# C-bowman/inference-tools

Measured on AMD Instinct MI355X. Metric: GpRegressor fit+predict wall-time and GFLOP/s at N=16384, d=8; % fp64 MFMA peak, higher is better.
Workload: dtype f64

## Files before the change

include/gpmi.h:

```cpp
#ifndef GPMI_H
#define GPMI_H

#include <stdint.h>

#ifdef __cplusplus
extern "C" {
#endif

#define GPMI_VERSION 100

#define GPMI_KERNEL_SE 0
#define GPMI_KERNEL_RQ 1
#define GPMI_KERNEL_SUM 2

#define GPMI_OK 0
#define GPMI_ERR_ARG (-1)
#define GPMI_ERR_HIP (-2)
#define GPMI_ERR_NOMEM (-3)
#define GPMI_ERR_NODEVICE (-4)
#define GPMI_ERR_INTERNAL (-5)

typedef struct gpmi_ctx gpmi_ctx;

int gpmi_version(void);
// ... 173 lines not shown
int gpmi_hdi_columns(gpmi_ctx* ctx, int64_t n, int64_t m, int64_t row_stride, int64_t col_stride,
                     const double* sample_host, int n_frac, const int64_t* L_host, int64_t ws_bytes,
                     double* hdi_host , int32_t* flag_host );

int gpmi_acf_columns(gpmi_ctx* ctx, int64_t n, int64_t m, int64_t row_stride, int64_t col_stride,
                     const double* sample_host, int64_t ws_bytes, double* f0_host , double* sum_host ,
                     int64_t* cut_host , int32_t* flag_host );
int gpmi_acf_lag_blocks(int64_t n, int64_t cap, int64_t* starts_host, int64_t* count);

int gpmi_timer_start(gpmi_ctx* ctx);
int gpmi_timer_stop(gpmi_ctx* ctx, float* ms);
int gpmi_flow_task_lists(int m, int nwg, int64_t cap, int32_t* out, int64_t* ntasks);

#define GPMI_PROF_KBUILD 0
#define GPMI_PROF_SYRK 1
#define GPMI_PROF_PANEL 2
#define GPMI_PROF_SOLVE 3
#define GPMI_PROF_SYRK_REST 4
#define GPMI_PROF_TRSM 5
#define GPMI_PROF_SYRK_SLICE 6
#define GPMI_PROF_FLOW 7
#define GPMI_PROF_NCLASS 8
int gpmi_profile_enable(gpmi_ctx* ctx, int on);
int gpmi_profile_read(gpmi_ctx* ctx, int klass, int64_t* launches, double* ms, double* flops,
                      double* bytes);
int gpmi_profile_reset(gpmi_ctx* ctx);
int gpmi_profile_clock(gpmi_ctx* ctx, double* ghz);

int gpmi_dev_alloc(gpmi_ctx* ctx, int64_t bytes, void** ptr_dev);
int gpmi_dev_free(gpmi_ctx* ctx, void* ptr_dev);
int gpmi_dev_upload(gpmi_ctx* ctx, void* dst_dev, const void* src_host, int64_t bytes);
int gpmi_dev_download(gpmi_ctx* ctx, void* dst_host, const void* src_dev, int64_t bytes);
int gpmi_dev_potrf(gpmi_ctx* ctx, double* A_dev, int64_t n, int64_t ld, int* info);
int gpmi_dev_gemm_nt(gpmi_ctx* ctx, double* C_dev, int64_t ldc, const double* A_dev, int64_t lda,
                     const double* B_dev, int64_t ldb, int64_t m, int64_t n, int64_t k, int lower);

#ifdef __cplusplus
}
#endif
#endif
```

inference-tools_amd/csrc/api.hip:

```cpp
#include "api_internal.h"
#include <malloc.h>


thread_local std::string g_create_err;


int lane_streams(gpmi_ctx* c, Lane& L) {
  const size_t index = c->lanes.size() - 1;
  L.owns_stream = index < 2;
  if (!L.owns_stream) L.stream = c->lanes[index % 2].stream;
  if (L.owns_stream) HIPCHK(c, hipStreamCreateWithFlags(&L.stream, hipStreamNonBlocking));
  hipDeviceProp_t prop;
  HIPCHK(c, hipGetDeviceProperties(&prop, c->device));
  c->ncu = prop.multiProcessorCount;
  HIPCHK(c, hipEventCreateWithFlags(&L.ev_la, hipEventDisableTiming));
  HIPCHK(c, hipEventCreateWithFlags(&L.ev_panel, hipEventDisableTiming));
  HIPCHK(c, hipEventCreateWithFlags(&L.ev_join, hipEventDisableTiming));
  HIPCHK(c, hipEventCreateWithFlags(&L.ev_main, hipEventDisableTiming));
  HIPCHK(c, hipEventCreateWithFlags(&L.ev_slice, hipEventDisableTiming));
  return GPMI_OK;
}


bool ensure_masked_pair(gpmi_ctx* c, Lane& L, int k) {
  (void)c;
  return L.sp[k] != nullptr && L.su[k] != nullptr;
}


int lane_masked_streams(gpmi_ctx* c, Lane& L) {
  const int ncu = c->ncu;
  if (ncu < 64 || ncu % 32 != 0) return GPMI_OK;
  for (int k = 0; k < GPMI_NPAIRS; ++k) {
    if (const char* e = std::getenv("GPMI_PANEL_CUS")) {
      const int v = std::atoi(e);
      if (v >= 8 && v <= ncu / 2 && v % 8 == 0) c->pair_cus[k] = v;
    }
    std::vector<uint32_t> panel((size_t)ncu / 32, 0u), upd((size_t)ncu / 32, 0xffffffffu);
    for (int i = 0; i < c->pair_cus[k]; ++i) {
      panel[(size_t)i / 32] |= 1u << (i % 32);
      upd[(size_t)i / 32] &= ~(1u << (i % 32));
    }
    hipError_t e1 = hipExtStreamCreateWithCUMask(&L.sp[k], (uint32_t)panel.size(), panel.data());
    hipError_t e2 = e1 == hipSuccess ? hipExtStreamCreateWithCUMask(&L.su[k], (uint32_t)upd.size(), upd.data()) : e1;
    if (e1 != hipSuccess || e2 != hipSuccess) {
      static bool told = false;
      if (!told) {
        told = true;
        std::fprintf(stderr, "[gpmi] a CU-masked stream pair could not be created (%s): this evaluation lane runs without "
                             "look-ahead and without the flag-ordered tail\n", hipGetErrorString(e1 != hipSuccess ? e1 : e2));
      }
      if (L.sp[k]) (void)hipStreamDestroy(L.sp[k]);
// ... 18 lines not shown
    }
    L.owns_pair = false;
  }
  const int64_t nt = c->np / GPMI_NB;
  HIPCHK(c, hipMalloc(&L.A, sizeof(double) * c->np * c->ld));
  HIPCHK(c, hipMalloc(&L.invD, sizeof(double) * nt * GPMI_NB * GPMI_NB));
  ZERO_SYNC(c, L.invD, sizeof(double) * nt * GPMI_NB * GPMI_NB);
  HIPCHK(c, hipMalloc(&L.vec, sizeof(double) * 4 * c->np));
  HIPCHK(c, hipMalloc(&L.red, sizeof(double) * 2 * RED_SLOTS));
  HIPCHK(c, hipMalloc(&L.info, sizeof(int) * RED_SLOTS));
  HIPCHK(c, hipHostMalloc(&L.h_red, sizeof(double) * 2 * RED_SLOTS));
  HIPCHK(c, hipHostMalloc(&L.h_info, sizeof(int) * RED_SLOTS));
  return GPMI_OK;
}

#define DBG_FREE(msg) do { if (std::getenv("GPMI_DEBUG_FREE")) std::fprintf(stderr, "[free] %s\n", msg); } while (0)
void lane_free(Lane& L) {
  DBG_FREE("lane: sync main stream");
  if (L.stream) (void)hipStreamSynchronize(L.stream);
  DBG_FREE("lane: sync masked streams");
  if (!L.owns_pair)
    for (int k = 0; k < GPMI_NPAIRS; ++k) L.sp[k] = L.su[k] = nullptr;
  for (int k = 0; k < GPMI_NPAIRS; ++k) {
    if (L.sp[k]) (void)hipStreamSynchronize(L.sp[k]);
    if (L.su[k]) (void)hipStreamSynchronize(L.su[k]);
  }
  potrf_flow_free(L);
  DBG_FREE("lane: destroy events");
  if (L.ev_la) (void)hipEventDestroy(L.ev_la);
  if (L.ev_panel) (void)hipEventDestroy(L.ev_panel);
  if (L.ev_join) (void)hipEventDestroy(L.ev_join);
  if (L.ev_main) (void)hipEventDestroy(L.ev_main);
  if (L.ev_slice) (void)hipEventDestroy(L.ev_slice);
  DBG_FREE("lane: destroy masked streams");
  if (L.sp[0] || L.su[0]) {
    static const int pause_ms = [] {
      const char* e = std::getenv("GPMI_DESTROY_PAUSE_MS");
      return e ? std::atoi(e) : 50;
    }();
    std::this_thread::sleep_for(std::chrono::milliseconds(pause_ms));
  }
  for (int k = 0; k < GPMI_NPAIRS; ++k) {
    if (L.sp[k]) (void)hipStreamDestroy(L.sp[k]);
    if (L.su[k]) (void)hipStreamDestroy(L.su[k]);
  }
  DBG_FREE("lane: free buffers");
  if (L.A) (void)hipFree(L.A);
  if (L.B2) (void)hipFree(L.B2);
  if (L.inv2) (void)hipFree(L.inv2);
  if (L.inv2_t) (void)hipFree(L.inv2_t);
  if (L.gws) (void)hipFree(L.gws);
  if (L.invD) (void)hipFree(L.invD);
  if (L.vec) (void)hipFree(L.vec);
  if (L.red) (void)hipFree(L.red);
  if (L.info) (void)hipFree(L.info);
  if (L.h_red) (void)hipHostFree(L.h_red);
  if (L.h_info) (void)hipHostFree(L.h_info);
  DBG_FREE("lane: destroy main stream");
  if (L.stream && L.owns_stream) (void)hipStreamDestroy(L.stream);
  DBG_FREE("lane: done");
  L = Lane();
}

int ensure_lanes(gpmi_ctx* c, size_t count) {
  while (c->lanes.size() < count) {
    c->lanes.emplace_back();
// ... 154 lines not shown
                     c->np, c->np, m > 0);
  }
  launch_add_diag_vec(s, dst, c->ld, c->noise, mx.extra, c->n);
}

int enqueue_factor_and_forward(gpmi_ctx* c, Lane& L, const CovParams& p, const double* mu_dev,
                               double mu_const, int slot, bool allow_lookahead,
                               const MixEval* mix, bool prebuild_inv2, double* backward_out, double* early_identity) {
  hipStream_t s = L.stream;
  L.inv2_valid = false;
  potrf_pair_quiesce(L);
  HIPCHK(c, hipMemsetAsync(L.info + slot, 0, sizeof(int), s));
  if (mix) {
    build_mix_square(c, s, *mix, L.A, false);
  } else {
    hipStream_t su = (!c->ycov && !((c->prof_mask >> GPMI_PROF_KBUILD) & 1))
                         ? potrf_first_update_stream(c, L, c->np, allow_lookahead)
                         : nullptr;
    static const bool no_split = std::getenv("GPMI_KBUILD_NO_SPLIT") != nullptr;
    if (su && !no_split) {
      HIPCHK(c, hipEventRecord(L.ev_join, s));
      HIPCHK(c, hipStreamWaitEvent(su, L.ev_join, 0));
      launch_kbuild_square_part(s, p, c->x, c->n, c->np, c->noise, L.A, c->ld, 1, GPMI_OB);
      launch_kbuild_square_part(su, p, c->x, c->n, c->np, c->noise, L.A, c->ld, 2, GPMI_OB);
    } else {
      ProfScope ps(c, s, GPMI_PROF_KBUILD, 0.0, 4.0 * c->np * c->np);
      launch_kbuild_square(s, p, c->x, c->n, c->np, c->noise, L.A, c->ld, true);
    }
  }
  if (c->ycov) launch_add_full(s, L.A, c->ld, c->ycov, c->n);
  static const bool early_fill = !std::getenv("GPMI_EARLY_FILL") || std::atoi(std::getenv("GPMI_EARLY_FILL")) != 0;
  L.early = Lane::EarlyWork();
  L.early.pending = true;
  L.early.y = c->y;
  L.early.mu = mu_dev;
  L.early.mu_const = mu_const;
  L.early.r = L.vec + 2 * c->np;
  L.early.n = c->n;
  L.early.np = c->np;
  L.early.fill[0] = L.vec;
  L.early.fill[1] = backward_out;
  L.early.ident = early_identity;
  L.early.ident_ld = c->ld;
  L.identity_ready = false;
  if (!early_fill) L.early.pending = false;
  potrf_lower(c, L, L.A, c->np, c->ld, L.invD, L.info + slot, allow_lookahead);
  if (!early_fill) L.early.pending = true;
  lane_run_early(L, s);
  if (prebuild_inv2 && L.su[0] && c->np >= 4 * GPMI_OB) {
    HIPCHK(c, hipEventRecord(L.ev_join, s));
    HIPCHK(c, hipStreamWaitEvent(L.su[0], L.ev_join, 0));
    if (int rc = ensure_inv2(c, L, L.su[0])) return rc;
    HIPCHK(c, hipEventRecord(L.ev_main, L.su[0]));
  }
  trsv_forward(c, s, L.A, c->np, c->ld, L.invD, L.vec + 2 * c->np, L.vec, L.info + slot, BatchShape(), true);
  if (prebuild_inv2 && L.inv2_valid && L.su[0]) {
    HIPCHK(c, hipEventRecord(L.ev_la, s));
    HIPCHK(c, hipStreamWaitEvent(L.su[0], L.ev_la, 0));
    launch_lml_reduce(L.su[0], L.vec, L.A, c->ld, c->np, L.red + 2 * slot);
    HIPCHK(c, hipEventRecord(L.ev_main, L.su[0]));
  } else {
    launch_lml_reduce(s, L.vec, L.A, c->ld, c->np, L.red + 2 * slot);
  }
  HIPCHK(c, hipGetLastError());
  return GPMI_OK;
}

int ensure_second_matrix(gpmi_ctx* c, Lane& L) {
  if (!L.B2) HIPCHK(c, hipMalloc(&L.B2, sizeof(double) * c->np * c->ld));
  return GPMI_OK;
}

int ensure_inv2(gpmi_ctx* c, Lane& F, hipStream_t s) {
  if (F.inv2_valid) return GPMI_OK;
  const int64_t nob = (c->np / GPMI_NB + 3) / 4;
  if (!F.inv2) HIPCHK(c, hipMalloc(&F.inv2, sizeof(double) * nob * GPMI_OB * GPMI_OB));
  if (!F.inv2_t) HIPCHK(c, hipMalloc(&F.inv2_t, sizeof(double) * nob * 256 * 256));
  build_inv2(s, F.A, c->np, c->ld, F.invD, F.inv2, F.inv2_t);
  HIPCHK(c, hipGetLastError());
  F.inv2_valid = true;
  return GPMI_OK;
}

int ensure_trsm_panel(gpmi_ctx* c, int64_t rows) {
  if (rows <= c->trsm_panel_rows) return GPMI_OK;
  if (c->trsm_panel) (void)hipFree(c->trsm_panel);
  c->trsm_panel = nullptr;
  c->trsm_panel_rows = 0;
// ... 549 lines not shown
    HIPCHK(c, hipMemcpyAsync(dbg + 22, &magic, sizeof(magic), hipMemcpyHostToDevice, s));
    launch_potrf_diag(s, A, ld, invD, dinfo, 0, dbg);
    std::vector<unsigned long long> hw(GPMI_STAMP_WORDS + TRACE_WORDS);
    HIPCHK(c, hipStreamSynchronize(s));
    HIPCHK(c, hipMemcpy(hw.data(), dbg, hw.size() * sizeof(unsigned long long), hipMemcpyDeviceToHost));
    const unsigned long long* h = hw.data() + 16;
    std::fprintf(stderr, "[potrf_diag] %.2f us | wave 0 cycles: load %llu | waits for its two tiles %llu | sub-diagonal panel + trailing tile %llu | end %llu | factor16 x8 %llu\n",
                 (double)(hw[8] - hw[0]) * 0.01, h[0], h[1], h[2], h[3], h[4]);
    for (int w = 0; w < 8; ++w) {
      if (w == 4) continue;
      std::fprintf(stderr, "[potrf_diag] wave %d (%s):", w, w == 0 ? "chain: start, W published, tiles seen, next block ready" : w < 4 ? "factor: start, W seen, panel done, panels seen, updates done" : "inverse: start, W seen, row done, operands seen, sums done");
      for (int k = 0; k < 9; ++k) {
        std::fprintf(stderr, " |");
        for (int e = 0; e < 6; ++e) {
          const unsigned long long v = hw[GPMI_STAMP_WORDS + (w * 9 + k) * 6 + e];
          if (v) std::fprintf(stderr, " %llu", v);
        }
      }
      std::fprintf(stderr, "\n");
    }
    (void)hipFree(dbg);
  } else
  potrf_lower(c, c->lanes[0], A, n, ld, invD, dinfo);
  int h = 0;
  hipError_t e = hipMemcpyAsync(&h, dinfo, sizeof(int), hipMemcpyDeviceToHost, s);
  if (e == hipSuccess) e = hipStreamSynchronize(s);
  (void)hipFree(invD);
  (void)hipFree(dinfo);
  HIPCHK(c, e);
  if (info) *info = h;
  return GPMI_OK;
}

int gpmi_dev_gemm_nt(gpmi_ctx* c, double* C, int64_t ldc, const double* A, int64_t lda,
                     const double* B, int64_t ldb, int64_t m, int64_t n, int64_t k, int lower) {
  if (!c) return GPMI_ERR_ARG;
  ARGCHK(c, m % GPMI_NB == 0 && n % GPMI_NB == 0 && k % 16 == 0 && m > 0 && n > 0 && k > 0,
         "m, n must be multiples of 128 and k of 16");
  if (int rc = set_device(c)) return rc;
  hipStream_t s;
  if (int rc = dev_stream(c, &s)) return rc;
  {
    const double tiles = lower ? (double)(n / GPMI_NB) * (n / GPMI_NB + 1) / 2.0 +
                                     (double)(m / GPMI_NB - n / GPMI_NB) * (n / GPMI_NB)
                               : (double)(m / GPMI_NB) * (n / GPMI_NB);
    unsigned long long* stamp =
        prof_stamp_slot(c, tiles * 2.0 * GPMI_NB * GPMI_NB * k, tiles * 16.0 * GPMI_NB * GPMI_NB);
    launch_gemm_nt(s, lower ? TILES_LOWER : TILES_RECT, OP_SUB, C, ldc, A, lda, B, ldb,
                   (int)(m / GPMI_NB), (int)(n / GPMI_NB), (int)k, stamp);
  }
  HIPCHK(c, hipGetLastError());
  HIPCHK(c, hipStreamSynchronize(s));
  return GPMI_OK;
}

}
```

inference-tools_amd/csrc/gpmi_internal.h:

```cpp
#pragma once
#include <hip/hip_runtime.h>
#include <cstdint>
#include <string>
#include <vector>

#include "gpmi.h"

constexpr int GPMI_NB = 128;
constexpr int GPMI_MAX_D = 64;
constexpr int GPMI_INFO_FLOW_TIMEOUT = -6;
constexpr int GPMI_NPAIRS = 1;

typedef double d2_t __attribute__((ext_vector_type(2)));
typedef double d4_t __attribute__((ext_vector_type(4)));

static inline int64_t round_up(int64_t v, int64_t m) { return (v + m - 1) / m * m; }

struct KParams {
  int kernel;
  int d;
  double a2;
  double kappa;
  double extra_diag;
  double inv_l2[GPMI_MAX_D];
};

constexpr int GPMI_MAX_SUM = 4;
struct CovParams : KParams {
  int nk = 0;
  KParams comp[GPMI_MAX_SUM] = {};
  CovParams() : KParams{} {}
  explicit CovParams(const KParams& k) : KParams(k) {}
};

struct ProfSlot {
  hipEvent_t e0, e1;
  int klass;
  double flops, bytes;
};

struct Lane {
  hipStream_t stream = nullptr;
  bool owns_stream = true;
  hipStream_t sp[GPMI_NPAIRS] = {nullptr};
  hipStream_t su[GPMI_NPAIRS] = {nullptr};
  bool owns_pair = true;
  struct EarlyWork {
    bool pending = false;
    const double* y = nullptr;
    const double* mu = nullptr;
    double mu_const = 0.0;
    double* r = nullptr;
    int64_t n = 0, np = 0;
    double* fill[2] = {nullptr, nullptr};
    double* ident = nullptr;
    int64_t ident_ld = 0;
  } early;
  bool identity_ready = false;
  bool pair_checked = false;
  hipEvent_t ev_la = nullptr, ev_panel = nullptr, ev_join = nullptr, ev_main = nullptr, ev_slice = nullptr;
  double* A = nullptr;
  double* invD = nullptr;
  double* B2 = nullptr;
  double* inv2 = nullptr;
  double* inv2_t = nullptr;
  bool inv2_valid = false;
  double* gws = nullptr;
  int64_t gws_doubles = 0;
  double* vec = nullptr;
  double* red = nullptr;
  int* info = nullptr;
  double* h_red = nullptr;
  int* h_info = nullptr;
  void* flow_tasks = nullptr;
  int* flow_off = nullptr;
  int* flow_flags = nullptr;
  int flow_m = 0, flow_nwg = 0, flow_nlists = 0;
  int64_t flow_ntasks = 0;
  double flow_flops_update = 0.0, flow_flops_trsm = 0.0;
};

struct LinvState {
  int64_t m = 0, mp = 0, ldm = 0;
  double* A = nullptr;
  double* At = nullptr;
  double* y = nullptr;
  double* sig2 = nullptr;
  double* zero = nullptr;
  double* K = nullptr;
  double* T = nullptr;
  double* J = nullptr;
  double* J2 = nullptr;
  double* Q = nullptr;
// ... 211 lines not shown
void launch_gemm_nt_range(hipStream_t s, GemmTiles tiles, GemmOp op, double* C, int64_t ldc, const double* A,
                          int64_t lda, const double* B, int64_t ldb, int ntr, int ntc, int k, int64_t first,
                          int64_t count, unsigned long long* stamp = nullptr);

void launch_gemm(hipStream_t s, GemmTiles tiles, GemmOp op, bool b_kmajor, int kskip, double* C,
                 int64_t ldc, const double* A, int64_t lda, const double* B, int64_t ldb, int ntr,
                 int ntc, int k, unsigned long long* stamp = nullptr, const GemmBatch& bt = GemmBatch());

hipStream_t potrf_first_update_stream(gpmi_ctx* c, Lane& lane, int64_t np, bool allow_lookahead);
void potrf_pair_quiesce(Lane& lane);
void launch_potrf_diag(hipStream_t s, double* Ablk, int64_t ld, double* invD, int* info, int col0,
                       unsigned long long* dbg = nullptr, const BatchShape& bs = BatchShape(), int* pub = nullptr,
                       int pub_val = 0);
void launch_potrf_diag_fault(hipStream_t s, double* Ablk, int64_t ld, const BatchShape& bs = BatchShape());
void potrf_lower_batched(gpmi_ctx* c, hipStream_t s, double* A, int64_t np, int64_t ld, double* invD,
                         int* info, const BatchShape& bs);
void launch_kbuild_square_batched(hipStream_t s, int kernel, const KParams* pdev, int batch, const double* x,
                                  int64_t n, int64_t np, const double* noise, double* A, int64_t ld,
                                  int64_t stride, int d, int64_t noise_stride = 0);
void potrf_lower(gpmi_ctx* c, Lane& lane, double* A, int64_t np, int64_t ld, double* invD,
                 int* info, bool allow_lookahead = true);

bool potrf_flow_enabled(gpmi_ctx* c, Lane& lane, int m);
bool potrf_flow_tail(gpmi_ctx* c, Lane& lane, double* A, int64_t ld, double* invD, int* info, int nt, int t0);
void potrf_flow_free(Lane& lane);

void trsv_forward(gpmi_ctx* c, hipStream_t s, const double* L, int64_t np, int64_t ld,
                  const double* invD, const double* r, double* out, int* err = nullptr,
                  const BatchShape& bs = BatchShape(), bool prefilled = false);
void trsv_backward(gpmi_ctx* c, hipStream_t s, const double* L, int64_t np, int64_t ld,
                   const double* invD, const double* r, double* out, int* err = nullptr,
                   const BatchShape& bs = BatchShape(), bool prefilled = false);
void lane_run_early(Lane& lane, hipStream_t s);
void trsm_identity_batched(hipStream_t s, const double* L, int64_t np, int64_t ld, const double* invD, double* Q,
                           const BatchShape& bs);
constexpr int GPMI_OB = 512;
void build_inv2(hipStream_t s, const double* L, int64_t np, int64_t ld, const double* invD, double* inv2,
                double* tmp);
void trsm_rows_forward(gpmi_ctx* c, hipStream_t s, const double* L, int64_t np, int64_t ld,
                       const double* inv2, double* Q, int64_t mp, bool upper_rhs, double* Qout,
                       double* panel);
void launch_set_identity(hipStream_t s, double* Q, int64_t ld, int64_t np, int batch = 1, int64_t sMat = 0);
void launch_copy(hipStream_t s, const double* src, double* dst, int64_t n);
void launch_copy_rows(hipStream_t s, const double* src, int64_t spitch, double* dst, int64_t dpitch, int64_t width,
                      int64_t height);
void launch_residual(hipStream_t s, const double* y, const double* mu, double mu_const, double* r,
                     int64_t n, int64_t np);
void launch_residual_batched(hipStream_t s, const double* y, const double* mus, const double* mu_consts,
                             double* r, int64_t n, int64_t np, const BatchShape& bs);
void launch_lml_reduce(hipStream_t s, const double* v, const double* L, int64_t ld, int64_t np,
                       double* red, const BatchShape& bs = BatchShape());
void launch_rows_dot(hipStream_t s, const double* Q, int64_t ld, int64_t mp, int64_t np,
                     const double* a, double* out, int batch = 1, int64_t sQ = 0, int64_t sVec = 0);
void launch_rows_sumsq(hipStream_t s, const double* Q, int64_t ld, int64_t mp, int64_t np,
                       double base, double* out, int batch = 1, int64_t sQ = 0, int64_t sVec = 0, double sign = 1.0);

void trsm_rows_backward(gpmi_ctx* c, hipStream_t s, const double* L, int64_t np, int64_t ld,
                        const double* invD, double* Q, int64_t mp, const double* inv2 = nullptr, double* panel = nullptr);

void launch_sd_reduce(hipStream_t s, const KParams& p, const double* x, int64_t n, const double* pts,
                      int64_t m, const double* Kq, int64_t ld, const double* W, int64_t ldw,
                      double scale, double* out);
void launch_grad_rhs(hipStream_t s, const KParams& p, const double* x, int64_t n, int64_t np,
                     const double* pts, int64_t rows_valid, int64_t rows_padded, const double* Kq,
                     int64_t ld, double* G);
void launch_grad_cov(hipStream_t s, const KParams& p, const double* G, int64_t ld, int64_t np,
// ... 2 lines not shown
```

inference-tools_amd/csrc/potrf.hip:

```cpp
#include <cstdlib>
#include <type_traits>
#include <utility>
#include <vector>

#include "gpmi_internal.h"
#include "potrf_diag.h"

namespace {

constexpr int NB = GPMI_NB;
using potrf_diag::DIAG_THREADS;

__global__ __launch_bounds__(DIAG_THREADS) void potrf_diag_kernel(double* __restrict__ A, int64_t ld,
                                                         double* __restrict__ invD,
                                                         int* __restrict__ info, int col0,
                                                         unsigned long long* __restrict__ dbg,
                                                         int64_t strideA, int64_t strideInv, int* pub, int pub_val) {
  if (pub && threadIdx.x == 0 && blockIdx.z == 0)
    __hip_atomic_store(pub, pub_val, __ATOMIC_RELAXED, __HIP_MEMORY_SCOPE_AGENT);
  __shared__ potrf_diag::DiagShared sh;
  potrf_diag::potrf_diag_body<false>(A + (int64_t)blockIdx.z * strideA, ld, invD + (int64_t)blockIdx.z * strideInv,
                                     info + blockIdx.z, col0, dbg, sh, potrf_diag::DiagPub());
}

}

namespace {
__global__ void fault_scale_kernel(double* A, int64_t ld, double f, int64_t strideA) {
  A += (int64_t)blockIdx.z * strideA;
  const int r = blockIdx.x, c = threadIdx.x;
  if (c <= r) A[(int64_t)r * ld + c] *= f;
}
}

void launch_potrf_diag_fault(hipStream_t s, double* Ablk, int64_t ld, const BatchShape& bs) {
  static const double fault = [] {
    const char* e = std::getenv("GPMI_FAULT_DIAG_EPS");
    return e ? std::atof(e) : 0.0;
  }();
  if (fault != 0.0)
    hipLaunchKernelGGL(fault_scale_kernel, dim3(NB, 1, (unsigned)bs.count), dim3(NB), 0, s, Ablk, ld, 1.0 + fault,
                       bs.sMat);
}

void launch_potrf_diag(hipStream_t s, double* Ablk, int64_t ld, double* invD, int* info, int col0,
                       unsigned long long* dbg, const BatchShape& bs, int* pub, int pub_val) {
  hipLaunchKernelGGL(potrf_diag_kernel, dim3(1, 1, (unsigned)bs.count), dim3(DIAG_THREADS), 0, s, Ablk, ld, invD,
                     info, col0, dbg, bs.sMat, bs.sInv, pub, pub_val);
  launch_potrf_diag_fault(s, Ablk, ld, bs);
}

namespace {

void factor_panel(gpmi_ctx* c, hipStream_t sp, double* A, int64_t ld, double* invD, int* info, int nt,
                  int J, int Je, int ncu = 0) {
  GemmBatch on;
  on.ncu_hint = ncu;
  on.b_lower_tri = true;
  static const bool trace = std::getenv("GPMI_CHAIN_TRACE") != nullptr;
  auto slot = [&](int tag) { return trace ? prof_stamp_slot(c, 0.0, 0.0, GPMI_PROF_NCLASS + tag) : nullptr; };
  for (int j = J; j < Je; ++j) {
    double* Ajj = A + (int64_t)j * NB * ld + (int64_t)j * NB;
    double* invDj = invD + (int64_t)j * NB * NB;
    const int below = nt - j - 1;
    {
      ProfScope ps(c, sp, GPMI_PROF_PANEL, (double)NB * NB * NB / 3.0 + 2.0 * below * NB * NB * NB,
                   8.0 * NB * NB * (2.0 + 2.0 * below));
      launch_potrf_diag(sp, Ajj, ld, invDj, info, j * NB, slot(0));
      if (below > 0) {
        double* A21 = Ajj + (int64_t)NB * ld;
        launch_gemm_nt(sp, TILES_RECT, OP_ASSIGN, A21, ld, A21, ld, invDj, NB, below, 1, NB, slot(1), on);
      }
    }
    const int pc = Je - j - 1;
    if (below > 0 && pc > 0) {
      double* A21 = Ajj + (int64_t)NB * ld;
      double* C = A21 + NB;
      const double tiles = pc * (pc + 1) / 2.0 + (double)(below - pc) * pc;
      ProfScope ps(c, sp, GPMI_PROF_PANEL, tiles * 2.0 * NB * NB * NB, tiles * 16.0 * NB * NB);
      launch_gemm_nt(sp, TILES_LOWER, OP_SUB, C, ld, A21, ld, A21, ld, below, pc, NB, slot(2));
    }
  }
}

void update_columns(gpmi_ctx* c, hipStream_t s, double* A, int64_t ld, int nt, int t0, int t1, int ka, int ke,
                    int ncu, int64_t slice = 0) {
  const int rows = nt - t0, cols = t1 - t0;
  const int kw = (ke - ka) * NB;
  if (rows <= 0 || cols <= 0 || kw <= 0) return;
  double* P = A + (int64_t)t0 * NB * ld + (int64_t)ka * NB;
  double* C = A + (int64_t)t0 * NB * ld + (int64_t)t0 * NB;
  const int64_t tiles = (int64_t)cols * (cols + 1) / 2 + (int64_t)(rows - cols) * cols - slice;
  const int64_t nfull = gemm_split_point(tiles, ncu, kw);
  static const int64_t BIG_MIN = [] {
    const char* e = std::getenv("GPMI_BIG_MIN");
    return (int64_t)(e ? std::atoi(e) : 384);
  }();
  const bool big = tiles >= BIG_MIN && kw > 128;
  int64_t nmain = big ? nfull : 0;
  if (big && nfull > 0 && nfull < tiles && gemm_mixed_launches()) nmain = tiles;
  unsigned long long* stamp = nullptr;
  unsigned long long* stamp_rest = nullptr;
  if (nmain > 0)
    stamp = prof_stamp_slot(c, (double)nmain * 2.0 * NB * NB * kw, (double)nmain * 16.0 * NB * NB + 8.0 * rows * NB * kw);
  if (tiles > nmain)
    stamp_rest = prof_stamp_slot(c, (double)(tiles - nmain) * 2.0 * NB * NB * kw, (double)(tiles - nmain) * 16.0 * NB * NB,
                                 GPMI_PROF_SYRK_REST);
  if (big)
    launch_gemm_nt_split(s, TILES_LOWER, OP_SUB, C, ld, P, ld, P, ld, rows, cols, kw, nfull, stamp, stamp_rest, tiles);
  else
    launch_gemm_nt_split(s, TILES_LOWER, OP_SUB, C, ld, P, ld, P, ld, rows, cols, kw, nfull, stamp_rest, nullptr, tiles);
// ... 22 lines not shown
  const double per_main = tile_us / (2.0 * ncu_main), per_panel = tile_us / (2.0 * ncu_panel);
  static const double CHAIN0 = [] {
    const char* e = std::getenv("GPMI_SLICE_CHAIN_US");
    return e ? std::atof(e) : 146.0;
  }();
  static const double SLOPE = [] {
    const char* e = std::getenv("GPMI_SLICE_CHAIN_SLOPE");
    return e ? std::atof(e) : 6.1;
  }();
  const double chain = CHAIN0 + SLOPE * rem;
  const double su = 20.0 + (double)(tiles_la + tiles_main) * per_main;
  double x = (su - chain) / (per_main + per_panel) * PCT / 100.0;
  const int64_t round = 2 * ncu_panel;
  int64_t n = x > 0 ? (int64_t)(x / round) * round : 0;
  const int64_t safe = tiles_main - (int64_t)8 * rem;
  if (n > safe) n = safe > 0 ? safe / round * round : 0;
  return n;
}

}

bool ensure_masked_pair(gpmi_ctx* c, Lane& L, int k);

namespace {
constexpr int OUTER_TILES = 4;
int lookahead_min() {
  static const int v = [] {
    const char* e = std::getenv("GPMI_LOOKAHEAD_MIN");
    const int x = e ? std::atoi(e) : 52;
    return x > 0 ? x : (1 << 30);
  }();
  return v;
}
}

void potrf_pair_quiesce(Lane& lane) {
  for (int k = 0; k < GPMI_NPAIRS; ++k)
    for (hipStream_t q : {lane.sp[k], lane.su[k]})
      if (q && hipStreamQuery(q) != hipSuccess) {
        (void)hipGetLastError();
        (void)hipStreamSynchronize(q);
      }
  lane.pair_checked = true;
}

hipStream_t potrf_first_update_stream(gpmi_ctx* c, Lane& lane, int64_t np, bool allow_lookahead) {
  const int nt = (int)(np / NB);
  if (!allow_lookahead || nt - OUTER_TILES < lookahead_min() || !ensure_masked_pair(c, lane, 0)) return nullptr;
  return lane.su[0];
}

void potrf_lower(gpmi_ctx* c, Lane& lane, double* A, int64_t np, int64_t ld, double* invD, int* info,
                 bool allow_lookahead) {
  hipStream_t sf = lane.stream;
  const int nt = (int)(np / NB);
  const int OBT = OUTER_TILES;
  const int LOOKAHEAD_MIN = lookahead_min();
  if (!lane.pair_checked) potrf_pair_quiesce(lane);
  lane.pair_checked = false;
  const bool la_ok = allow_lookahead && nt - OBT >= LOOKAHEAD_MIN && ensure_masked_pair(c, lane, 0);
  const bool flow_ok = allow_lookahead;
  if (flow_ok && !(la_ok && nt - OBT >= LOOKAHEAD_MIN) && potrf_flow_enabled(c, lane, nt) &&
      potrf_flow_tail(c, lane, A, ld, invD, info, nt, 0))
    return;
  auto follow = [](hipStream_t waiter, hipStream_t producer, hipEvent_t ev) {
    if (waiter != producer) (void)hipStreamWaitEvent(waiter, ev, 0);
  };
  auto tile0 = [&](int panel) { return panel * OBT < nt ? panel * OBT : nt; };
  const int NP = (nt + OBT - 1) / OBT;
  factor_panel(c, sf, A, ld, invD, info, nt, 0, tile0(1));
  hipStream_t panel_stream = sf;
  hipStream_t main_stream = sf;
  bool sliced = false;
  (void)hipEventRecord(lane.ev_panel, sf);
  (void)hipEventRecord(lane.ev_main, sf);
  if (la_ok && NP > 1 && nt - tile0(1) >= LOOKAHEAD_MIN) lane_run_early(lane, sf);
  for (int p = 0; p + 1 < NP; ++p) {
    const int k0 = tile0(p), k1 = tile0(p + 1);
    const int rem = nt - k1;
    const bool overlap = la_ok && rem >= LOOKAHEAD_MIN;
    hipStream_t su = overlap ? lane.su[0] : sf, sp = overlap ? lane.sp[0] : sf;
    const int ncu = overlap ? c->ncu - c->pair_cus[0] : c->ncu;
    follow(su, panel_stream, lane.ev_panel);
    follow(su, main_stream, lane.ev_main);
    int64_t slice = 0;
    if (overlap) {
      const int k2 = tile0(p + 2);
      update_columns(c, su, A, ld, nt, k1, k2, k0, k1, ncu);
      (void)hipEventRecord(lane.ev_la, su);
      (void)hipStreamWaitEvent(sp, lane.ev_la, 0);
      const int w = k2 - k1, r2 = nt - k2;
      slice = slice_tiles(rem, (int64_t)w * (w + 1) / 2 + (int64_t)(rem - w) * w, (int64_t)r2 * (r2 + 1) / 2,
                          (k1 - k0) * NB, ncu, c->pair_cus[0]);
      if (sliced) (void)hipStreamWaitEvent(su, lane.ev_slice, 0);
      update_columns(c, su, A, ld, nt, k2, nt, k0, k1, ncu, slice);
      (void)hipEventRecord(lane.ev_main, su);
    } else {
      if (sliced) (void)hipStreamWaitEvent(su, lane.ev_slice, 0);
      update_columns(c, su, A, ld, nt, k1, nt, k0, k1, ncu);
      if (flow_ok && potrf_flow_enabled(c, lane, nt - k1) && potrf_flow_tail(c, lane, A, ld, invD, info, nt, k1)) return;
    }
    sliced = false;
    main_stream = su;
    factor_panel(c, sp, A, ld, invD, info, nt, k1, tile0(p + 2), overlap ? c->pair_cus[0] : 0);
    if (overlap) (void)hipEventRecord(lane.ev_panel, sp);
    panel_stream = sp;
    if (slice > 0) {
      update_slice(c, sp, A, ld, nt, tile0(p + 2), nt, k0, k1, slice);
      (void)hipEventRecord(lane.ev_slice, sp);
      sliced = true;
    }
  }
  follow(sf, panel_stream, lane.ev_panel);
  follow(sf, main_stream, lane.ev_main);
  if (sliced) (void)hipStreamWaitEvent(sf, lane.ev_slice, 0);
}

void potrf_lower_batched(gpmi_ctx* c, hipStream_t s, double* A, int64_t np, int64_t ld, double* invD,
                         int* info, const BatchShape& bs) {
  (void)c;
  static const int OBT = [] {
    const char* e = std::getenv("GPMI_BATCH_OUTER");
    const int v = e ? std::atoi(e) : 4;
    return v > 0 ? v : 1;
  }();
  const int nt = (int)(np / NB);
  GemmBatch inplace{bs.count, bs.sMat, bs.sMat, bs.sInv};
  inplace.b_lower_tri = true;
  const GemmBatch upd{bs.count, bs.sMat, bs.sMat, bs.sMat};
  static const bool left = [] {
    const char* e = std::getenv("GPMI_BATCH_LEFT");
    return !e || std::atoi(e) != 0;
  }();
  for (int J = 0; J < nt; J += OBT) {
    const int Je = (J + OBT < nt) ? J + OBT : nt;
    for (int j = J; j < Je; ++j) {
      double* Ajj = A + (int64_t)j * NB * ld + (int64_t)j * NB;
      double* invDj = invD + (int64_t)j * NB * NB;
      const int below = nt - j - 1;
      if (left && j > J) {
        const double* P = A + (int64_t)j * NB * ld + (int64_t)J * NB;
        launch_gemm_nt(s, TILES_LOWER, OP_SUB, Ajj, ld, P, ld, P, ld, nt - j, 1, (j - J) * NB, nullptr, upd);
      }
      launch_potrf_diag(s, Ajj, ld, invDj, info, j * NB, nullptr, bs);
// ... 17 lines not shown
```

inference-tools_amd/csrc/solve.hip:

```cpp
#include <cstdlib>
#include <mutex>

#include "gpmi_internal.h"

namespace {

constexpr int NB = GPMI_NB;

__device__ inline double wave_sum(double v) {
#pragma unroll
  for (int off = 32; off > 0; off >>= 1) v += __shfl_down(v, off, 64);
  return v;
}

constexpr unsigned long long FLOW_SENTINEL = 0xFFF8DEADBEEF0000ull;
constexpr int FLOW_THREADS = 512;
constexpr int FLOW_SPIN_LIMIT = 1 << 22;

__device__ inline double flow_poll(const double* p, int* err, bool& dead) {
  const unsigned long long* q = reinterpret_cast<const unsigned long long*>(p);
  unsigned long long bits = __hip_atomic_load(q, __ATOMIC_RELAXED, __HIP_MEMORY_SCOPE_AGENT);
  int spins = 0;
  while (bits == FLOW_SENTINEL && !dead) {
    __builtin_amdgcn_s_sleep(1);
// ... 370 lines not shown
  }
  s = wave_sum(s);
  if (lane == 0) out[row] = sign * (base - s);
}

}

constexpr int64_t FLOW_GATE_MIN = 32;
namespace {
std::mutex g_sweep_mu;
hipEvent_t g_sweep_ev[64] = {nullptr};
bool g_sweep_used[64] = {false};
}
static void flow_gate_enter(gpmi_ctx* c, hipStream_t s, int64_t workgroups) {
  if (workgroups <= FLOW_GATE_MIN || c->device < 0 || c->device >= 64) return;
  std::lock_guard<std::mutex> lk(g_sweep_mu);
  const int d = c->device;
  if (!g_sweep_ev[d] && hipEventCreateWithFlags(&g_sweep_ev[d], hipEventDisableTiming) != hipSuccess) {
    g_sweep_ev[d] = nullptr;
    (void)hipGetLastError();
    return;
  }
  if (g_sweep_used[d]) (void)hipStreamWaitEvent(s, g_sweep_ev[d], 0);
}
static void flow_gate_leave(gpmi_ctx* c, hipStream_t s, int64_t workgroups) {
  if (workgroups <= FLOW_GATE_MIN || c->device < 0 || c->device >= 64) return;
  std::lock_guard<std::mutex> lk(g_sweep_mu);
  const int d = c->device;
  if (!g_sweep_ev[d]) return;
  (void)hipEventRecord(g_sweep_ev[d], s);
  g_sweep_used[d] = true;
}

void lane_run_early(Lane& lane, hipStream_t s) {
  Lane::EarlyWork& e = lane.early;
  if (!e.pending) return;
  e.pending = false;
  launch_residual(s, e.y, e.mu, e.mu_const, e.r, e.n, e.np);
  for (double* f : e.fill)
    if (f) hipLaunchKernelGGL(flow_fill_kernel, dim3((unsigned)((e.np + 255) / 256), 1, 1), dim3(256), 0, s, f, e.np, (int64_t)0);
  if (e.ident) {
    launch_set_identity(s, e.ident, e.ident_ld, e.np);
    lane.identity_ready = true;
  }
}

void trsv_forward(gpmi_ctx* c, hipStream_t s, const double* L, int64_t np, int64_t ld,
                  const double* invD, const double* r, double* out, int* err, const BatchShape& bs, bool prefilled) {
  const int nt = (int)(np / NB);
  flow_gate_enter(c, s, (int64_t)nt);
  ProfScope ps(c, s, GPMI_PROF_SOLVE, (double)np * np, 4.0 * np * np);
  if (!prefilled)
    hipLaunchKernelGGL(flow_fill_kernel, dim3((unsigned)((np + 255) / 256), 1, (unsigned)bs.count), dim3(256), 0, s,
                       out, np, bs.sVec);
  const unsigned grid = bs.count > 1 ? 8u * (unsigned)nt * (unsigned)((bs.count + 7) / 8) : (unsigned)nt;
  hipLaunchKernelGGL(trsv_fwd_flow_kernel, dim3(grid), dim3(FLOW_THREADS), 0, s, L, ld, invD, r, out, err, bs.sMat,
                     bs.sInv, bs.sVec, nt, bs.count);
  flow_gate_leave(c, s, (int64_t)nt);
}

void trsv_backward(gpmi_ctx* c, hipStream_t s, const double* L, int64_t np, int64_t ld,
                   const double* invD, const double* r, double* out, int* err, const BatchShape& bs, bool prefilled) {
  const int nt = (int)(np / NB);
  flow_gate_enter(c, s, (int64_t)nt);
  ProfScope ps(c, s, GPMI_PROF_SOLVE, (double)np * np, 4.0 * np * np);
  if (!prefilled)
    hipLaunchKernelGGL(flow_fill_kernel, dim3((unsigned)((np + 255) / 256), 1, (unsigned)bs.count), dim3(256), 0, s, out,
                       np, bs.sVec);
  const unsigned grid = bs.count > 1 ? 8u * (unsigned)nt * (unsigned)((bs.count + 7) / 8) : (unsigned)nt;
  hipLaunchKernelGGL(trsv_bwd_flow_kernel, dim3(grid), dim3(FLOW_THREADS), 0, s, L, ld, invD, r, out, err, nt, bs.sMat,
                     bs.sInv, bs.sVec, bs.count);
  flow_gate_leave(c, s, (int64_t)nt);
}

void build_inv2(hipStream_t s, const double* L, int64_t np, int64_t ld, const double* invD, double* inv2,
                double* tmp) {
  const int nt = (int)(np / NB);
// ... 168 lines not shown
```

inference-tools_amd/inference_amd/_lib.py:

```python
import atexit
import ctypes as C
import os
import sys
import weakref

import numpy as np

_HERE = os.path.dirname(os.path.abspath(__file__))
LIB_PATH = os.environ.get("GPMI_LIB") or os.path.join(_HERE, "lib", "libgpmi.so")

KERNEL_SE = 0
KERNEL_RQ = 1
KERNEL_SUM = 2
PROF_KBUILD, PROF_SYRK, PROF_PANEL, PROF_SOLVE, PROF_SYRK_REST, PROF_TRSM, PROF_SYRK_SLICE, PROF_FLOW = 0, 1, 2, 3, 4, 5, 6, 7
OPT_LOCKSTEP_ALWAYS, OPT_RESERVE_POINTS, OPT_NO_FLOW = 1, 2, 3
PREDICT_PANEL = 256
_TRACE_MS = float(os.environ["GPMI_TRACE_CALLS"]) if os.environ.get("GPMI_TRACE_CALLS") else None
ERR_INTERNAL = -5


class GpmiUnavailable(RuntimeError):
    """libgpmi.so (the HIP extension) or an MI355X device is missing."""


# ... 72 lines not shown
    "gpmi_comm_allgather": (C.c_int, [_vp, _dp, _dp, _i64]),
    "gpmi_comm_broadcast": (C.c_int, [_vp, _dp, _i64, C.c_int]),
    "gpmi_comm_count": (C.c_int, [_vp, C.POINTER(C.c_int)]),
    "gpmi_comm_destroy": (C.c_int, [_vp]),
    "gpmi_kde_create": (C.c_int, [_vp, _i64, _dp, _i64, C.POINTER(_i64), C.POINTER(_i64), C.POINTER(_vp)]),
    "gpmi_kde_destroy": (C.c_int, [_vp]),
    "gpmi_kde_eval": (C.c_int, [_vp, _i64, _dp, C.POINTER(_i64), C.c_double, _dp, _dp]),
    "gpmi_kde_cv_logprob": (C.c_int, [_vp, _i64, _dp, C.c_int, _dp, C.c_double, _dp]),
    "gpmi_kde2d_create": (C.c_int, [_vp, _i64, _dp, _dp, C.POINTER(_vp)]),
    "gpmi_kde2d_destroy": (C.c_int, [_vp, _vp]),
    "gpmi_kde2d_eval": (C.c_int, [_vp, _vp, _i64, _dp, _dp, C.c_double, C.c_double, _dp]),
    "gpmi_kde2d_self": (C.c_int, [_vp, _vp, C.c_double, C.c_double, _dp, C.POINTER(_i64)]),
    "gpmi_kde2d_grid": (C.c_int, [_vp, _vp, _i64, _dp, _i64, _dp, C.c_double, C.c_double, _dp]),
    "gpmi_unimodal_create": (C.c_int, [_vp, _i64, _dp, C.POINTER(_vp)]),
    "gpmi_unimodal_destroy": (C.c_int, [_vp, _vp]),
    "gpmi_unimodal_logpdf_sums": (C.c_int, [_vp, _vp, _i64, C.c_int, _dp, _dp]),
    "gpmi_hdi_columns": (C.c_int, [_vp, _i64, _i64, _i64, _i64, _dp, C.c_int, C.POINTER(_i64), _i64, _dp,
                                   C.POINTER(C.c_int32)]),
    "gpmi_acf_columns": (C.c_int, [_vp, _i64, _i64, _i64, _i64, _dp, _i64, _dp, _dp, C.POINTER(_i64),
                                   C.POINTER(C.c_int32)]),
    "gpmi_acf_lag_blocks": (C.c_int, [_i64, _i64, C.POINTER(_i64), C.POINTER(_i64)]),
    "gpmi_timer_start": (C.c_int, [_vp]),
    "gpmi_timer_stop": (C.c_int, [_vp, C.POINTER(C.c_float)]),
    "gpmi_profile_enable": (C.c_int, [_vp, C.c_int]),
    "gpmi_profile_read": (C.c_int, [_vp, C.c_int, C.POINTER(_i64), _dp, _dp, _dp]),
    "gpmi_profile_reset": (C.c_int, [_vp]),
    "gpmi_profile_clock": (C.c_int, [_vp, _dp]),
    "gpmi_dev_alloc": (C.c_int, [_vp, _i64, C.POINTER(_vp)]),
    "gpmi_dev_free": (C.c_int, [_vp, _vp]),
    "gpmi_dev_upload": (C.c_int, [_vp, _vp, _vp, _i64]),
    "gpmi_dev_download": (C.c_int, [_vp, _vp, _vp, _i64]),
    "gpmi_dev_potrf": (C.c_int, [_vp, _vp, _i64, _i64, _ip]),
    "gpmi_dev_gemm_nt": (C.c_int, [_vp, _vp, _i64, _vp, _i64, _vp, _i64, _i64, _i64, _i64, C.c_int]),
}

_lib = None


def load():
    global _lib
    if _lib is None:
        if not os.path.exists(LIB_PATH):
            raise GpmiUnavailable(
                f"{LIB_PATH} not found - build the HIP extension first "
                "(python -c 'import __graft_entry__ as g; g.build()' or make -C inference-tools_amd/csrc)"
            )
        lib = C.CDLL(LIB_PATH)
        for name, (res, args) in SIGNATURES.items():
            fn = getattr(lib, name)
            fn.restype = res
            fn.argtypes = args
        _lib = lib
        atexit.register(_close_all_handles)
    return _lib


def device_count() -> int:
    cnt = C.c_int(0)
    load().gpmi_device_count(C.byref(cnt))
    return cnt.value


def device_identity(device: int) -> str:
    buf = C.create_string_buffer(64)
    rc = load().gpmi_device_pci_bus_id(int(device), buf, 64)
    return buf.value.decode() if rc == 0 else ""
# ... 89 lines not shown
```

Before: 54920.

## Overlap forward triangular solve with Cholesky panels and split lookahead update

Adds a panel-forward kernel that solves the right-hand side against each finished Cholesky panel and updates the residual for the rows below. It runs on the factorization streams while later panels are still being factored, so the trailing forward trsv only covers the unfinished tiles. It also splits the lookahead column update so the next panel can start after its first tile column is ready, waiting on the rest later. This adds extra kernels, events and cross-stream dependencies, which brings synchronization overhead and a risk of ordering errors.

```diff
diff --git a/include/gpmi.h b/include/gpmi.h
--- a/include/gpmi.h
+++ b/include/gpmi.h
@@ -229,6 +229,9 @@
 int gpmi_dev_upload(gpmi_ctx* ctx, void* dst_dev, const void* src_host, int64_t bytes);
 int gpmi_dev_download(gpmi_ctx* ctx, void* dst_host, const void* src_dev, int64_t bytes);
 int gpmi_dev_potrf(gpmi_ctx* ctx, double* A_dev, int64_t n, int64_t ld, int* info);
+int gpmi_dev_panel_forward(gpmi_ctx* ctx, const double* L_dev, int64_t ld, const double* invD_dev, double* r_dev,
+                           double* z_dev, int64_t nt, int64_t k0, int64_t w, int64_t row_first, int64_t row_count,
+                           int store_z);
 int gpmi_dev_gemm_nt(gpmi_ctx* ctx, double* C_dev, int64_t ldc, const double* A_dev, int64_t lda,
                      const double* B_dev, int64_t ldb, int64_t m, int64_t n, int64_t k, int lower);
 
diff --git a/inference-tools_amd/csrc/api.hip b/inference-tools_amd/csrc/api.hip
--- a/inference-tools_amd/csrc/api.hip
+++ b/inference-tools_amd/csrc/api.hip
@@ -18,6 +18,8 @@
   HIPCHK(c, hipEventCreateWithFlags(&L.ev_join, hipEventDisableTiming));
   HIPCHK(c, hipEventCreateWithFlags(&L.ev_main, hipEventDisableTiming));
   HIPCHK(c, hipEventCreateWithFlags(&L.ev_slice, hipEventDisableTiming));
+  HIPCHK(c, hipEventCreateWithFlags(&L.ev_la_rest, hipEventDisableTiming));
+  HIPCHK(c, hipEventCreateWithFlags(&L.ev_fwd, hipEventDisableTiming));
   return GPMI_OK;
 }
 
@@ -102,6 +104,8 @@
   if (L.ev_join) (void)hipEventDestroy(L.ev_join);
   if (L.ev_main) (void)hipEventDestroy(L.ev_main);
   if (L.ev_slice) (void)hipEventDestroy(L.ev_slice);
+  if (L.ev_la_rest) (void)hipEventDestroy(L.ev_la_rest);
+  if (L.ev_fwd) (void)hipEventDestroy(L.ev_fwd);
   DBG_FREE("lane: destroy masked streams");
   if (L.sp[0] || L.su[0]) {
     static const int pause_ms = [] {
@@ -322,6 +326,7 @@
   static const bool early_fill = !std::getenv("GPMI_EARLY_FILL") || std::atoi(std::getenv("GPMI_EARLY_FILL")) != 0;
   L.early = Lane::EarlyWork();
   L.early.pending = true;
+  L.early.residual_pending = true;
   L.early.y = c->y;
   L.early.mu = mu_dev;
   L.early.mu_const = mu_const;
@@ -334,6 +339,10 @@
   L.early.ident_ld = c->ld;
   L.identity_ready = false;
   if (!early_fill) L.early.pending = false;
+  L.fwd = Lane::FwdShadow();
+  L.fwd.armed = true;
+  L.fwd.r = L.vec + 2 * c->np;
+  L.fwd.out = L.vec;
   potrf_lower(c, L, L.A, c->np, c->ld, L.invD, L.info + slot, allow_lookahead);
   if (!early_fill) L.early.pending = true;
   lane_run_early(L, s);
@@ -343,7 +352,13 @@
     if (int rc = ensure_inv2(c, L, L.su[0])) return rc;
     HIPCHK(c, hipEventRecord(L.ev_main, L.su[0]));
   }
-  trsv_forward(c, s, L.A, c->np, c->ld, L.invD, L.vec + 2 * c->np, L.vec, L.info + slot, BatchShape(), true);
+  {
+    const int64_t ft = L.fwd.done_tiles, off = ft * GPMI_NB;
+    if (ft > 0) HIPCHK(c, hipStreamWaitEvent(s, L.ev_fwd, 0));
+    if (off < c->np)
+      trsv_forward(c, s, L.A + off * c->ld + off, c->np - off, c->ld, L.invD + ft * GPMI_NB * GPMI_NB,
+                   L.vec + 2 * c->np + off, L.vec + off, L.info + slot, BatchShape(), ft == L.fwd.plan_tiles);
+  }
   if (prebuild_inv2 && L.inv2_valid && L.su[0]) {
     HIPCHK(c, hipEventRecord(L.ev_la, s));
     HIPCHK(c, hipStreamWaitEvent(L.su[0], L.ev_la, 0));
@@ -959,6 +974,21 @@
   return GPMI_OK;
 }
 
+int gpmi_dev_panel_forward(gpmi_ctx* c, const double* L, int64_t ld, const double* invD, double* r, double* z,
+                           int64_t nt, int64_t k0, int64_t w, int64_t row_first, int64_t row_count, int store_z) {
+  if (!c) return GPMI_ERR_ARG;
+  ARGCHK(c, L && invD && r && z && ld >= nt * GPMI_NB && ld % 2 == 0, "bad matrix shape");
+  ARGCHK(c, k0 >= 0 && w >= 1 && w <= 4 && k0 + w <= nt, "the panel must be 1 .. 4 tile columns inside the matrix");
+  ARGCHK(c, row_count >= 0 && row_first >= k0 + w && row_first + row_count <= nt, "rows must lie below the panel");
+  if (int rc = set_device(c)) return rc;
+  hipStream_t s;
+  if (int rc = dev_stream(c, &s)) return rc;
+  launch_panel_forward(c, s, L, ld, invD, r, z, (int)k0, (int)w, (int)row_first, (int)row_count, store_z != 0);
+  HIPCHK(c, hipGetLastError());
+  HIPCHK(c, hipStreamSynchronize(s));
+  return GPMI_OK;
+}
+
 int gpmi_dev_gemm_nt(gpmi_ctx* c, double* C, int64_t ldc, const double* A, int64_t lda,
                      const double* B, int64_t ldb, int64_t m, int64_t n, int64_t k, int lower) {
   if (!c) return GPMI_ERR_ARG;
diff --git a/inference-tools_amd/csrc/gpmi_internal.h b/inference-tools_amd/csrc/gpmi_internal.h
--- a/inference-tools_amd/csrc/gpmi_internal.h
+++ b/inference-tools_amd/csrc/gpmi_internal.h
@@ -52,13 +52,22 @@
     double mu_const = 0.0;
     double* r = nullptr;
     int64_t n = 0, np = 0;
+    bool residual_pending = false;
     double* fill[2] = {nullptr, nullptr};
     double* ident = nullptr;
     int64_t ident_ld = 0;
   } early;
+  struct FwdShadow {
+    bool armed = false;
+    double* r = nullptr;
+    double* out = nullptr;
+    int plan_tiles = 0, done_tiles = 0;
+  } fwd;
+  hipEvent_t ev_fwd = nullptr;
   bool identity_ready = false;
   bool pair_checked = false;
   hipEvent_t ev_la = nullptr, ev_panel = nullptr, ev_join = nullptr, ev_main = nullptr, ev_slice = nullptr;
+  hipEvent_t ev_la_rest = nullptr;
   double* A = nullptr;
   double* invD = nullptr;
   double* B2 = nullptr;
@@ -336,6 +345,9 @@
                    const double* invD, const double* r, double* out, int* err = nullptr,
                    const BatchShape& bs = BatchShape(), bool prefilled = false);
 void lane_run_early(Lane& lane, hipStream_t s);
+void lane_run_residual(Lane& lane, hipStream_t s);
+void launch_panel_forward(gpmi_ctx* c, hipStream_t s, const double* L, int64_t ld, const double* invD, double* r,
+                          double* z, int k0, int w, int row_first, int row_count, bool store_z);
 void trsm_identity_batched(hipStream_t s, const double* L, int64_t np, int64_t ld, const double* invD, double* Q,
                            const BatchShape& bs);
 constexpr int GPMI_OB = 512;
diff --git a/inference-tools_amd/csrc/potrf.hip b/inference-tools_amd/csrc/potrf.hip
--- a/inference-tools_amd/csrc/potrf.hip
+++ b/inference-tools_amd/csrc/potrf.hip
@@ -53,7 +53,7 @@
 namespace {
 
 void factor_panel(gpmi_ctx* c, hipStream_t sp, double* A, int64_t ld, double* invD, int* info, int nt,
-                  int J, int Je, int ncu = 0) {
+                  int J, int Je, int ncu = 0, hipEvent_t rest_ready = nullptr) {
   GemmBatch on;
   on.ncu_hint = ncu;
   on.b_lower_tri = true;
@@ -77,6 +77,7 @@
       double* A21 = Ajj + (int64_t)NB * ld;
       double* C = A21 + NB;
       const double tiles = pc * (pc + 1) / 2.0 + (double)(below - pc) * pc;
+      if (rest_ready && j == J) (void)hipStreamWaitEvent(sp, rest_ready, 0);
       ProfScope ps(c, sp, GPMI_PROF_PANEL, tiles * 2.0 * NB * NB * NB, tiles * 16.0 * NB * NB);
       launch_gemm_nt(sp, TILES_LOWER, OP_SUB, C, ld, A21, ld, A21, ld, below, pc, NB, slot(2));
     }
@@ -165,6 +166,20 @@
   }();
   return v;
 }
+bool fwd_shadow_on() {
+  static const bool v = [] {
+    const char* e = std::getenv("GPMI_FWD_SHADOW");
+    return !e || std::atoi(e) != 0;
+  }();
+  return v;
+}
+int la_split_mode() {
+  static const int v = [] {
+    const char* e = std::getenv("GPMI_LA_SPLIT");
+    return e ? std::atoi(e) : 1;
+  }();
+  return v;
+}
 }
 
 void potrf_pair_quiesce(Lane& lane) {
@@ -189,6 +204,10 @@
   const int nt = (int)(np / NB);
   const int OBT = OUTER_TILES;
   const int LOOKAHEAD_MIN = lookahead_min();
+  Lane::FwdShadow& fw = lane.fwd;
+  const bool fwd_armed = fw.armed && fw.r && fw.out && fwd_shadow_on();
+  fw.armed = false;
+  fw.plan_tiles = fw.done_tiles = 0;
   if (!lane.pair_checked) potrf_pair_quiesce(lane);
   lane.pair_checked = false;
   const bool la_ok = allow_lookahead && nt - OBT >= LOOKAHEAD_MIN && ensure_masked_pair(c, lane, 0);
@@ -201,6 +220,18 @@
   };
   auto tile0 = [&](int panel) { return panel * OBT < nt ? panel * OBT : nt; };
   const int NP = (nt + OBT - 1) / OBT;
+  if (fwd_armed && la_ok)
+    for (int p = 0; p + 1 < NP && nt - tile0(p + 1) >= LOOKAHEAD_MIN; ++p) fw.plan_tiles = tile0(p + 2);
+  hipStream_t fwd_stream = nullptr;
+  auto forward_panel = [&](hipStream_t s, hipStream_t factored_on, int q) {
+    const int a = tile0(q), b = tile0(q + 1);
+    follow(s, factored_on, lane.ev_panel);
+    if (fwd_stream) follow(s, fwd_stream, lane.ev_fwd);
+    launch_panel_forward(c, s, A, ld, invD, fw.r, fw.out, a, b - a, b, nt - b, true);
+    (void)hipEventRecord(lane.ev_fwd, s);
+    fwd_stream = s;
+    fw.done_tiles = b;
+  };
   factor_panel(c, sf, A, ld, invD, info, nt, 0, tile0(1));
   hipStream_t panel_stream = sf;
   hipStream_t main_stream = sf;
@@ -208,6 +239,10 @@
   (void)hipEventRecord(lane.ev_panel, sf);
   (void)hipEventRecord(lane.ev_main, sf);
   if (la_ok && NP > 1 && nt - tile0(1) >= LOOKAHEAD_MIN) lane_run_early(lane, sf);
+  if (fw.plan_tiles > 0) {
+    lane_run_residual(lane, sf);
+    forward_panel(sf, sf, 0);
+  }
   for (int p = 0; p + 1 < NP; ++p) {
     const int k0 = tile0(p), k1 = tile0(p + 1);
     const int rem = nt - k1;
@@ -217,14 +252,20 @@
     follow(su, panel_stream, lane.ev_panel);
     follow(su, main_stream, lane.ev_main);
     int64_t slice = 0;
+    bool split = false;
     if (overlap) {
       const int k2 = tile0(p + 2);
-      update_columns(c, su, A, ld, nt, k1, k2, k0, k1, ncu);
-      (void)hipEventRecord(lane.ev_la, su);
-      (void)hipStreamWaitEvent(sp, lane.ev_la, 0);
       const int w = k2 - k1, r2 = nt - k2;
       slice = slice_tiles(rem, (int64_t)w * (w + 1) / 2 + (int64_t)(rem - w) * w, (int64_t)r2 * (r2 + 1) / 2,
                           (k1 - k0) * NB, ncu, c->pair_cus[0]);
+      split = w > 1 && (la_split_mode() >= 2 || (la_split_mode() == 1 && slice == 0));
+      update_columns(c, su, A, ld, nt, k1, split ? k1 + 1 : k2, k0, k1, ncu);
+      (void)hipEventRecord(lane.ev_la, su);
+      (void)hipStreamWaitEvent(sp, lane.ev_la, 0);
+      if (split) {
+        update_columns(c, su, A, ld, nt, k1 + 1, k2, k0, k1, ncu);
+        (void)hipEventRecord(lane.ev_la_rest, su);
+      }
       if (sliced) (void)hipStreamWaitEvent(su, lane.ev_slice, 0);
       update_columns(c, su, A, ld, nt, k2, nt, k0, k1, ncu, slice);
       (void)hipEventRecord(lane.ev_main, su);
@@ -235,7 +276,8 @@
     }
     sliced = false;
     main_stream = su;
-    factor_panel(c, sp, A, ld, invD, info, nt, k1, tile0(p + 2), overlap ? c->pair_cus[0] : 0);
+    factor_panel(c, sp, A, ld, invD, info, nt, k1, tile0(p + 2), overlap ? c->pair_cus[0] : 0,
+                 split ? lane.ev_la_rest : nullptr);
     if (overlap) (void)hipEventRecord(lane.ev_panel, sp);
     panel_stream = sp;
     if (slice > 0) {
@@ -243,6 +285,7 @@
       (void)hipEventRecord(lane.ev_slice, sp);
       sliced = true;
     }
+    if (overlap && fw.done_tiles < fw.plan_tiles) forward_panel(tile0(p + 2) < fw.plan_tiles ? sf : sp, sp, p + 1);
   }
   follow(sf, panel_stream, lane.ev_panel);
   follow(sf, main_stream, lane.ev_main);
diff --git a/inference-tools_amd/csrc/solve.hip b/inference-tools_amd/csrc/solve.hip
--- a/inference-tools_amd/csrc/solve.hip
+++ b/inference-tools_amd/csrc/solve.hip
@@ -426,17 +426,97 @@
   g_sweep_used[d] = true;
 }
 
+void lane_run_residual(Lane& lane, hipStream_t s) {
+  Lane::EarlyWork& e = lane.early;
+  if (!e.residual_pending) return;
+  e.residual_pending = false;
+  launch_residual(s, e.y, e.mu, e.mu_const, e.r, e.n, e.np);
+}
+
 void lane_run_early(Lane& lane, hipStream_t s) {
   Lane::EarlyWork& e = lane.early;
   if (!e.pending) return;
   e.pending = false;
-  launch_residual(s, e.y, e.mu, e.mu_const, e.r, e.n, e.np);
-  for (double* f : e.fill)
-    if (f) hipLaunchKernelGGL(flow_fill_kernel, dim3((unsigned)((e.np + 255) / 256), 1, 1), dim3(256), 0, s, f, e.np, (int64_t)0);
+  lane_run_residual(lane, s);
+  for (int k = 0; k < 2; ++k) {
+    const int64_t off = (k == 0 && e.fill[0] == lane.fwd.out) ? (int64_t)lane.fwd.plan_tiles * NB : 0;
+    if (e.fill[k] && off < e.np)
+      hipLaunchKernelGGL(flow_fill_kernel, dim3((unsigned)((e.np - off + 255) / 256), 1, 1), dim3(256), 0, s, e.fill[k] + off,
+                         e.np - off, (int64_t)0);
+  }
   if (e.ident) {
     launch_set_identity(s, e.ident, e.ident_ld, e.np);
     lane.identity_ready = true;
   }
+}
+
+constexpr int PF_THREADS = 512;
+constexpr int PF_MAXW = 4;
+
+__device__ inline void pf_rows_dot(const double* __restrict__ M, int64_t ld, int ntile, const double* x, double* y) {
+  const int lane = threadIdx.x & 63, wave = threadIdx.x >> 6;
+  double acc[16];
+#pragma unroll
+  for (int i = 0; i < 16; ++i) acc[i] = 0.0;
+  const double* base = M + (int64_t)(wave * 16) * ld + 2 * lane;
+  for (int t = 0; t < ntile; ++t) {
+    const d2_t xv = *reinterpret_cast<const d2_t*>(x + t * NB + 2 * lane);
+    d2_t a[16];
+#pragma unroll
+    for (int i = 0; i < 16; ++i) a[i] = *reinterpret_cast<const d2_t*>(base + (int64_t)i * ld + (int64_t)t * NB);
+#pragma unroll
+    for (int i = 0; i < 16; ++i) acc[i] = fma(a[i][0], xv[0], fma(a[i][1], xv[1], acc[i]));
+  }
+#pragma unroll
+  for (int i = 0; i < 16; ++i) {
+    const double sum = wave_sum(acc[i]);
+    if (lane == 0) y[wave * 16 + i] = sum;
+  }
+}
+
+__global__ __launch_bounds__(PF_THREADS) void panel_forward_kernel(const double* __restrict__ L, int64_t ld,
+                                                                  const double* __restrict__ invD, double* r,
+                                                                  double* __restrict__ z, int k0, int w, int row_first,
+                                                                  int row_count) {
+  __shared__ __attribute__((aligned(16))) double zs[PF_MAXW * NB];
+  __shared__ __attribute__((aligned(16))) double u[NB];
+  __shared__ double y[NB];
+  const int tid = threadIdx.x;
+  for (int j = 0; j < w; ++j) {
+    const int kj = k0 + j;
+    if (j > 0) {
+      pf_rows_dot(L + (int64_t)kj * NB * ld + (int64_t)k0 * NB, ld, j, zs, y);
+      __syncthreads();
+    }
+    if (tid < NB) {
+      const double rj = r[(int64_t)kj * NB + tid];
+      u[tid] = j > 0 ? rj - y[tid] : rj;
+    }
+    __syncthreads();
+    pf_rows_dot(invD + (int64_t)kj * NB * NB, NB, 1, u, y);
+    __syncthreads();
+    if (tid < NB) zs[j * NB + tid] = y[tid];
+    __syncthreads();
+  }
+  if ((int)blockIdx.x < row_count) {
+    const int i = row_first + (int)blockIdx.x;
+    pf_rows_dot(L + (int64_t)i * NB * ld + (int64_t)k0 * NB, ld, w, zs, y);
+    __syncthreads();
+    if (tid < NB) r[(int64_t)i * NB + tid] -= y[tid];
+  } else {
+    for (int t = tid; t < w * NB; t += PF_THREADS) z[(int64_t)k0 * NB + t] = zs[t];
+  }
+}
+
+void launch_panel_forward(gpmi_ctx* c, hipStream_t s, const double* L, int64_t ld, const double* invD, double* r,
+                          double* z, int k0, int w, int row_first, int row_count, bool store_z) {
+  const unsigned grid = (unsigned)row_count + (store_z ? 1u : 0u);
+  if (grid == 0 || w < 1 || w > PF_MAXW) return;
+  const double cols = (double)w * NB;
+  ProfScope ps(c, s, GPMI_PROF_SOLVE, 2.0 * row_count * NB * cols + (double)grid * cols * cols,
+               8.0 * row_count * NB * cols + 4.0 * (double)grid * cols * cols);
+  hipLaunchKernelGGL(panel_forward_kernel, dim3(grid), dim3(PF_THREADS), 0, s, L, ld, invD, r, z, k0, w, row_first,
+                     row_count);
 }
 
 void trsv_forward(gpmi_ctx* c, hipStream_t s, const double* L, int64_t np, int64_t ld,
diff --git a/inference-tools_amd/inference_amd/_lib.py b/inference-tools_amd/inference_amd/_lib.py
--- a/inference-tools_amd/inference_amd/_lib.py
+++ b/inference-tools_amd/inference_amd/_lib.py
@@ -128,6 +128,7 @@
     "gpmi_dev_download": (C.c_int, [_vp, _vp, _vp, _i64]),
     "gpmi_dev_potrf": (C.c_int, [_vp, _vp, _i64, _i64, _ip]),
     "gpmi_dev_gemm_nt": (C.c_int, [_vp, _vp, _i64, _vp, _i64, _vp, _i64, _i64, _i64, _i64, C.c_int]),
+    "gpmi_dev_panel_forward": (C.c_int, [_vp, _vp, _i64, _vp, _vp, _vp, _i64, _i64, _i64, _i64, _i64, C.c_int]),
 }
 
 _lib = None
```

Result: slower. 54230 (-1.3%).
